# flydog-sdr/FlyDog_SDR_GPS

Measured on AMD Instinct MI355X. Metric: IQ Msamples/s ingested (waterfall + GPS acq); value = GPS acq, BASELINE configs[1], higher is better.
Workload: dtype f32

## Files before the change

### flydog_sdr_gps_amd/_lib.py

```python
import ctypes as C
import os

import numpy as np

_HERE = os.path.dirname(os.path.abspath(__file__))
_LIB = None

ABI_VERSION = 4


class KiwiGpuError(RuntimeError):
    def __init__(self, status, where, text):
        super().__init__("%s failed: %s (status %d)" % (where, text, status))
        self.status = status


def library_path():
    return os.environ.get("KIWIGPU_LIBRARY") or os.path.join(_HERE, "libkiwigpu.so")


class AcqResultC(C.Structure):
    _fields_ = [("snr", C.c_float), ("dop", C.c_int32), ("idx", C.c_int32), ("valid", C.c_int32)]


# ... 253 lines not shown
    "kg_rxbank_set_wf": (_i, [_vp, _i, C.c_uint64, _i, _i]),
    "kg_rxbank_set_wf_pkt": (_i, [_vp, _i, C.c_uint32, C.c_uint32, _i]),
    "kg_rxbank_set_unpack": (_i, [_vp, C.c_float, C.c_float, C.c_float, _i]),
    "kg_rxbank_step": (_i, [_vp, _vp, _vp, _vp]),
    "kg_rxbank_adc_done": (_i, [_vp, _vp, _i]),
    "kg_snd_iq_payload_dev": (_i, [_vp, _vp, _i, _vp, _sz, _i, _i, _vp, _sz]),
    "kg_rxbank_set_little_endian": (_i, [_vp, _i, _i]),
    "kg_post_get_mode": (_i, [_vp, _i]),
    "kg_math_dev": (_i, [_vp, _i, C.c_float, _vp, C.c_uint32, C.c_size_t, _vp]),
    "kg_math_atan2f_dev": (_i, [_vp, _vp, _vp, C.c_size_t, _vp]),
    "kg_rxbank_poll": (_i, [_vp]),
    "kg_rxbank_ready": (_i, [_vp]),
    "kg_rxbank_join": (_i, [_vp, _i]),
    "kg_rxbank_leave": (_i, [_vp, _i]),
    "kg_rxbank_is_active": (_i, [_vp, _i]),
    "kg_rxbank_audio_map": (_i, [_vp, _vp, _vp, _vp, _vp]),
    "kg_fir_process_each_dev": (_i, [_vp, _vp, _i, _vp, _sz, _vp, _vp, _sz, _vp]),
    "kg_rxbank_sync": (_i, [_vp]),
    "kg_rxbank_frame_map": (_i, [_vp, _vp, _vp, _vp]),
    "kg_rxbank_buffers": (_i, [_vp, _vp]),
    "kg_rxbank_host_profile": (_i, [_vp, C.c_char_p, _sz]),
    "kg_acq_debug_fft_stamps": (_i, [_vp, _i, _vp, _i]),
    "kg_acq_debug_corr_stamps": (_i, [_vp, _i, _vp, _i, _vp, _i]),
}


def _share_hip_runtime_with_torch():
    import sys
    if "torch" in sys.modules or os.environ.get("KIWIGPU_NO_TORCH_PRELOAD") == "1":
        return
    import importlib.util
    if importlib.util.find_spec("torch") is not None:
        try:
            import torch
        except Exception as e:
            import warnings
            warnings.warn("kiwigpu: torch is installed but failed to import (%s: %s); libkiwigpu.so will use "
                          "the system HIP runtime" % (type(e).__name__, e))


def load_library():
    global _LIB
    if _LIB is not None:
        return _LIB
    path = library_path()
    if not os.path.exists(path):
# ... 138 lines not shown
```

### flydog_sdr_gps_amd/acq.py

```python
import ctypes as C
from collections import namedtuple

import numpy as np

from . import sats as _sats
from . import prn as _prn
from ._lib import Context, cell_dtype, check, ptr, result_dtype

NSAMPLES = 65536
FFT_LEN = 16384
DECIM = 4
BIN_SIZE = 249.755859375
NSAMPLES_10MS = 163680
FFT_LEN_10MS = 65536
BIN_SIZE_10MS = 4.092e6 / 65536
DOP_LO, DOP_HI = -20, 20
MIN_SIG = 16

AcqResult = namedtuple("AcqResult", "sat snr lo_shift ca_shift valid")


class Searcher:

    def __init__(self, ctx=None, max_sats=_sats.MAX_SATS, dop_lo=DOP_LO, dop_hi=DOP_HI,
# ... 119 lines not shown
        self._last = (int(nblocks), sats.size)

    def fetch(self, want_cells=True):
        nb, ns = self._last
        res = np.zeros((nb, ns), result_dtype)
        cells = np.zeros((nb, ns, self.ndop), cell_dtype) if want_cells else None
        check(self.lib.kg_acq_fetch(self.h, ptr(res), ptr(cells)), "kg_acq_fetch")
        return res, cells

    def correlate_many(self, sats, nblocks=1, want_cells=True, first_block=0):
        self.correlate_async(sats, nblocks, first_block)
        return self.fetch(want_cells)

    def correlate(self, sat, block_data=None):
        if block_data is not None:
            self.set_data_fft(block_data, 0)
        res, _ = self.correlate_many([sat], 1, want_cells=False)
        r = res[0, 0]
        return float(r["snr"]), int(r["dop"]), int(r["idx"]), int(r["valid"])

    def results_dev(self):
        return self.lib.kg_acq_results_dev(self.h)

    def search(self, sats, packed=None, iq16=None, lo_shift=0, ca_shift=0):
        if packed is not None:
            self.sample(packed)
        elif iq16 is not None:
            self.sample_iq16(iq16)
        res, _ = self.correlate_many(list(sats), 1, want_cells=False)
        out = []
        for sat, r in zip(sats, res[0]):
            if r["valid"]:
                lo_shift, ca_shift = int(r["dop"]), int(r["idx"]) * DECIM
            out.append(AcqResult(int(sat), float(r["snr"]), lo_shift, ca_shift, int(r["valid"])))
        return out
```

### flydog_sdr_gps_amd/csrc/kg_acq.hip

```cpp
#include "kg_common.h"
#include "kg_fft.h"
#include "kg_acq_tables.h"

#include <math.h>
#include <stdlib.h>
#include <vector>

#define SUB      4096
#define NTAPS    31
#define DECIM    4


enum { SRC_BITS = 0, SRC_IQ16 = 1, SRC_CHIPS = 2 };

__constant__ float c_hb_even[16] = {
    -0.010233f,  0.010668f, -0.016324f,  0.024377f, -0.036482f,  0.056990f, -0.101993f,
     0.316926f,  0.316926f, -0.101993f,  0.056990f, -0.036482f,  0.024377f, -0.016324f,
     0.010668f, -0.010233f,
};
#define HB_CENTRE 0.500009f

KG_DEV float bipolar(int bit) { return bit ? -1.0f : 1.0f; }

template <int SRC>
KG_DEV cf acq_source(const void *__restrict__ src, int i, int nvalid, int nchips, int boc)
// ... 149 lines not shown
    }
}

struct acq_red { float p; int i; float s; int pad; };

#define ACQ_CLAIM_STRIDE 32
#define ACQ_LDS_BYTES (2 * SUB * sizeof(float2) + 16)

struct __attribute__((aligned(16))) acq_part { float p; int i; float s; int pad; };

struct acq_pair_desc {
    int data_off;
    int code_off;
    int limit;
    int out;
};

struct acq_cell_desc { int data_off, code_off, dop, limit, out; };

struct acq_walk {
    int npairs;
    int ndop, dop_lo;
};

template <int P, bool STAMPS = false>
__global__ __launch_bounds__(256, 2) void acq_correlate_kernel(
    const float2 *__restrict__ data,
    const float2 *__restrict__ code,
    const float2 *__restrict__ tab4096, const float2 *__restrict__ tabN,
    const float2 *__restrict__ comb,
    const acq_pair_desc *__restrict__ pairs,
    int *__restrict__ claim,
    acq_walk walk,
    int halo,
    acq_part *__restrict__ parts,
    unsigned long long *__restrict__ stamps = nullptr)
{
    static_assert(P == 4 || P == 16, "N = 16384 or 65536");
    constexpr int LOGP = P == 4 ? 2 : 4;
    extern __shared__ __attribute__((aligned(16))) float2 smem[];
    float2 *tileA = smem, *tileB = smem + SUB;
    typedef __attribute__((address_space(3))) volatile int acq_lds_int;
    acq_lds_int *claim_slot = (acq_lds_int *) (smem + 2 * SUB);
    const int t = threadIdx.x;
    unsigned long long *st = (STAMPS && t == 0 && blockIdx.x == 8) ? stamps : nullptr;
    if (STAMPS && st) { st[0] = __builtin_amdgcn_s_memtime(); st[1] = __builtin_amdgcn_s_memrealtime(); }
    unsigned long long *wgt = (STAMPS && t == 0) ? stamps + 512 + 4 * blockIdx.x : nullptr;
    int wg_cells = 0;
    if (STAMPS && wgt) {
        wgt[0] = __builtin_amdgcn_s_memrealtime();
        wgt[2] = (unsigned long long) __builtin_amdgcn_s_getreg((20 << 0) | (0 << 6) | (31 << 11));
    }

    kg_tw4096 tw;
    kg_tw4096_load(tw, tab4096, t);
    cf V[4];
#pragma unroll
    for (int dd = 0; dd < 4; dd++) V[dd] = kg_ld(&tabN[t + 1024 * dd]);

    const int xcd = blockIdx.x & 7, slot = blockIdx.x >> 3, nslots = gridDim.x >> 3;
    const int gpairs = (walk.npairs - xcd + 7) >> 3;
    const bool spread = walk.npairs < 8;
    const int ndop = walk.ndop, ncell = spread ? (walk.npairs * ndop - xcd + 7) >> 3 : gpairs * ndop;

    typedef unsigned u4 __attribute__((ext_vector_type(4)));
    const int rowb_c = 2 * (256 + 2 * halo) * (int) sizeof(float2);
    const int plane_c = 8 * 2 * (256 + 2 * halo);
    cf d[16], c[16];
    struct acq_rsrc { __amdgpu_buffer_rsrc_t drs, crs; int dvo, cvo; };
    auto fetch_prepare = [&](int data_off, int code_off, int dop, int k2) {
        const int s = k2 - dop;
        const int q0 = s >> LOGP;
        acq_rsrc r;
        r.drs = __builtin_amdgcn_make_buffer_rsrc(
            (void *) (data + data_off + k2 * SUB), 0, SUB * (int) sizeof(float2), 0x00020000);
        r.crs = __builtin_amdgcn_make_buffer_rsrc(
            (void *) (code + code_off + (s & (P - 1)) * plane_c), 0, plane_c * (int) sizeof(float2), 0x00020000);
        r.dvo = t * 16; r.cvo = (t + q0 + halo) * 16;
        return r;
    };
    auto fetch_row = [&](const acq_rsrc &r, int i) {
        const u4 dv = __builtin_amdgcn_raw_buffer_load_b128(r.drs, r.dvo, i * 4096, 0);
        const u4 cv = __builtin_amdgcn_raw_buffer_load_b128(r.crs, r.cvo, i * rowb_c, 0);
        d[2 * i] = cf{__uint_as_float(dv[0]), __uint_as_float(dv[1])};
// ... 1 lines not shown
        c[2 * i] = cf{__uint_as_float(cv[0]), __uint_as_float(cv[1])};
        c[2 * i + 1] = cf{__uint_as_float(cv[2]), __uint_as_float(cv[3])};
    };
    auto fetch_drow = [&](const acq_rsrc &r, int i) {
        int so;
        asm volatile("s_mov_b32 %0, %1" : "=s"(so) : "i"(i * 4096));
        const u4 dv = __builtin_amdgcn_raw_buffer_load_b128(r.drs, r.dvo, so, 0);
        d[2 * i] = cf{__uint_as_float(dv[0]), __uint_as_float(dv[1])};
        d[2 * i + 1] = cf{__uint_as_float(dv[2]), __uint_as_float(dv[3])};
    };
    auto fetch_crow = [&](const acq_rsrc &r, int i) {
        const u4 cv = __builtin_amdgcn_raw_buffer_load_b128(r.crs, r.cvo, i * rowb_c, 0);
        c[2 * i] = cf{__uint_as_float(cv[0]), __uint_as_float(cv[1])};
        c[2 * i + 1] = cf{__uint_as_float(cv[2]), __uint_as_float(cv[3])};
    };
    auto fetch = [&](int data_off, int code_off, int dop, int k2) {
        const acq_rsrc r = fetch_prepare(data_off, code_off, dop, k2);
#pragma unroll
        for (int i = 0; i < 8; i++) fetch_row(r, i);
    };
    auto describe = [&](int idx) {
        const int cell = spread ? (idx << 3) + xcd : idx;
        const int pg = cell / ndop, di = cell - pg * ndop;
        const acq_pair_desc pd = pairs[spread ? pg : (pg << 3) + xcd];
        return acq_cell_desc{pd.data_off, pd.code_off, walk.dop_lo + di, pd.limit, pd.out + di};
    };

    int cur_idx = slot, nxt_idx = slot + nslots;
    if (cur_idx >= ncell) return;
    acq_cell_desc cur = describe(cur_idx);
    fetch(cur.data_off, cur.code_off, cur.dop, P - 1);

    if (t == 0) claim_slot[1] = slot + 2 * nslots;
    int par = 0;

    int st_item = 0;
    for (;;) {
        const bool more = nxt_idx < ncell;
        const acq_cell_desc nxt = describe(more ? nxt_idx : cur_idx);
        int claimed = 0;
        if (t == 0) claimed = __hip_atomic_fetch_add(&claim[xcd * ACQ_CLAIM_STRIDE], 1, __ATOMIC_RELAXED, __HIP_MEMORY_SCOPE_AGENT);
        cf acc[16];
        cf yprev[16];
        auto accumulate = [&](cf (&yv)[16], bool first, bool mid = false) {
            if (first) {
#pragma unroll
                for (int m = 0; m < 16; m++) acc[m] = yv[m];
// ... 120 lines not shown
                    bp = take ? pw : bp; br = take ? m : br;
                    sum += pw;
                } else {
                    const bool in = t + 256 * m < limit, take = in & (pw > bp);
                    bp = take ? pw : bp; br = take ? m : br;
                    sum += in ? pw : 0.f;
                }
            }
            bi = t + 256 * br;
        }
        {
            float wmax = bp, wsum = sum;
            kg_wave_max_sum(wmax, wsum);
            const int wn = kg_wave_min(bp == wmax ? bi : 0x7fffffff);
            if ((t & 63) == 0) parts[4 * cur.out + (t >> 6)] = acq_part{wmax, wn, wsum, 0};
        }
        if (t == 0) claim_slot[par] = 3 * nslots + claimed;
        const int nn_idx = __builtin_amdgcn_readfirstlane(claim_slot[par ^ 1]);
        par ^= 1;
        if (STAMPS) wg_cells++;
        if (!more) break;
        cur = nxt; cur_idx = nxt_idx; nxt_idx = nn_idx;
    }
    if (STAMPS && st) { st[2] = __builtin_amdgcn_s_memtime(); st[3] = __builtin_amdgcn_s_memrealtime(); }
    if (STAMPS && wgt) { wgt[1] = __builtin_amdgcn_s_memrealtime(); wgt[3] = (unsigned long long) wg_cells; }
}

#define ACQ8_LDS_BYTES (3 * SUB * sizeof(float2) + 8 * sizeof(acq_red) + 16 + 16 * 8 * sizeof(float2) + 3 * 512 * 4)


template <int P, bool STAMPS = false>
__global__ __launch_bounds__(512, 1) void acq_correlate8_kernel(
    const float2 *__restrict__ data, const float2 *__restrict__ code,
    const float2 *__restrict__ tab4096, const float2 *__restrict__ tabN,
    const float2 *__restrict__ comb8,
    const float2 *__restrict__ quart,
    const acq_pair_desc *__restrict__ pairs, int *__restrict__ claim, acq_walk walk, int halo,
    kg_acq_cell *__restrict__ cells, unsigned long long *__restrict__ stamps = nullptr)
{
    static_assert(P == 4 || P == 16, "N = 16384 or 65536");
    constexpr int LOGP = P == 4 ? 2 : 4;
    extern __shared__ __attribute__((aligned(16))) float2 smem[];
    float2 *tile0 = smem, *tile1 = smem + SUB, *tile2 = smem + 2 * SUB;
    acq_red *red = (acq_red *) (smem + 3 * SUB);
    volatile int *red_claim = (volatile int *) (red + 8);
    float2 *cst = (float2 *) ((char *) (red + 8) + 16);
// ... 274 lines not shown
        int bi = i + 512 * (int) __builtin_ctz(rowmask | 0x80000000u);
        KG_STAMP(STAMPS, stc, 1);
        xch_p[i] = bp; xch_i[i] = bi; xch_s[i] = sum;
        KG_STAMP(STAMPS, stc, 2);
        if (i == 448) *red_claim = 2 * nslots + claimed;
        __syncthreads();
        KG_STAMP(STAMPS, stc, 3);
        const int nn_idx = __builtin_amdgcn_readfirstlane(*red_claim);
        prev_out = cur.out; prev_limit = limit;
        if (!more) {
            reduce_pairs();
            __syncthreads();
            merge_store(prev_out, prev_limit);
        }
        KG_STAMP(STAMPS, stc, 4);
        if (!more) break;
        cur = nxt; cur_idx = nxt_idx; nxt_idx = nn_idx;
    }
}

__global__ __launch_bounds__(64) void acq_select_kernel(kg_acq_cell *__restrict__ cells, const acq_part *__restrict__ parts,
                                                       const acq_pair_desc *__restrict__ pairs, int np1,
                                                       int npairs, int dop_lo, int ndop,
                                                       kg_acq_result *__restrict__ out, int *__restrict__ claim)
{
    const int q = blockIdx.x, lane = threadIdx.x;
    if (q == 0 && lane < 16) claim[lane * ACQ_CLAIM_STRIDE] = 0;
    if (q >= npairs) return;
    const acq_pair_desc pd = pairs[q];
    const int p = pd.out / ndop;
    float bs = 0.f;
    int bd = 0x7fffffff, bidx = 0;
    for (int di = lane; di < ndop; di += 64) {
        kg_acq_cell c;
        if (q < np1) {
            const acq_part *w = parts + 4 * ((size_t) pd.out + di);
            acq_part a = w[0], b = w[2];
            const acq_part a1 = w[1], b1 = w[3];
            auto merge = [](acq_part &x, const acq_part &o) {
                const bool take = (o.p > x.p) | ((o.p == x.p) & (o.i < x.i));
                x.p = take ? o.p : x.p; x.i = take ? o.i : x.i;
                x.s += o.s;
            };
            merge(a, a1); merge(b, b1); merge(a, b);
            const float ave = a.s / (float) pd.limit;
            c.snr = a.p / ave;
            c.max_pwr = a.p; c.tot_pwr = a.s; c.idx = a.i;
            cells[(size_t) pd.out + di] = c;
        } else {
            c = cells[(size_t) pd.out + di];
// ... 40 lines not shown
    kg_dbuf<float2> d_fsub;
    kg_dbuf<float2> d_fsub_code;
    kg_dbuf<uint8_t> d_in;
    kg_hbuf<uint8_t> h_pin[4];
    hipEvent_t ev_pin[4];
    int pin_next;
    kg_hbuf<uint8_t> h_batch; size_t batch_cap; hipEvent_t ev_batch;
    hipStream_t cstream; hipEvent_t ev_in_free; bool in_free_set;
    kg_dbuf<uint8_t> d_chips;
    kg_dbuf<kg_acq_cell> d_cells;
    kg_dbuf<acq_part> d_parts;
    kg_dbuf<kg_acq_result> d_results;
    kg_dbuf<int> d_claim;
    std::vector<int> limits, code_set;
    std::vector<int> last_sats;
    const acq_pair_desc *d_pairs1, *d_pairs4;
    unsigned long pairs_seq;
    int last_first, last_nblocks, last_nsats, np1, np4, table_nblocks;
    hipStream_t fstream;
    bool own_fstream;
    std::vector<hipEvent_t> ev_ready, ev_done;
    std::vector<int> ready_of, done_of;
    int grid1;
};

static inline __host__ __device__ size_t plane_pos(int k1, int halo_col, int H, int layout)
{
    if (layout == 0) {
        const int t = k1 & 255, j = k1 >> 8, row = 2 * (256 + 2 * H);
        return (size_t) (j >> 1) * row + 2 * (t + halo_col + H) + (j & 1);
    }
    const int t = k1 & 511, j = k1 >> 9, row = 2 * (512 + 2 * H);
    return (size_t) (j >> 1) * row + 2 * (t + halo_col + H) + (j & 1);
}
static inline size_t spec_len(int P, int H) { return (size_t) P * 8 * 2 * (256 + 2 * H); }
static inline __host__ __device__ size_t plane_len(int H, int layout) { return layout == 0 ? (size_t) 8 * 2 * (256 + 2 * H) : (size_t) 4 * 2 * (512 + 2 * H); }

__global__ void acq_code_overrun_kernel(float2 *__restrict__ dst, int layout_dst, const float2 *__restrict__ src, int layout_src, int P, int H)
{
    const int t = blockIdx.x * blockDim.x + threadIdx.x;
    if (t >= P * H) return;
    const int k2 = t % P, k1 = t / P;
    const float2 v = src ? src[(size_t) k2 * plane_len(H, layout_src) + plane_pos(k1, 0, H, layout_src)] : make_float2(0.f, 0.f);
    const int T = layout_dst == 0 ? 256 : 512, J = SUB / T;
    dst[(size_t) k2 * plane_len(H, layout_dst) + plane_pos(k1 + T * (J - 1), T, H, layout_dst)] = v;
}

// ... 91 lines not shown
        KG_TRY(a->d_comb8.alloc(comb8.size(), "kg_acq_create: combine constants"));
        KG_HIP(hipMemcpy(a->d_comb8, comb8.data(), sizeof(float2) * comb8.size(), hipMemcpyHostToDevice));
    }
    KG_TRY(a->d_code.alloc(a->code_len * max_sats, "kg_acq_create: code spectra"));
    KG_TRY(a->d_data.alloc((size_t) N * max_blocks, "kg_acq_create: data spectra"));
    KG_TRY(a->d_td.alloc((size_t) N * max_blocks, "kg_acq_create: decimated samples"));
    KG_TRY(a->d_td_code.alloc(N, "kg_acq_create: decimated samples"));
    KG_TRY(a->d_fsub.alloc((size_t) N * max_blocks, "kg_acq_create: sub-transforms"));
    KG_TRY(a->d_fsub_code.alloc(N, "kg_acq_create: sub-transforms"));
    KG_TRY(a->d_in.alloc(a->in_stride * max_blocks, "kg_acq_create: input staging"));
    for (int k = 0; k < 4; k++) {
        KG_TRY(a->h_pin[k].alloc(a->in_stride, "kg_acq_create: pinned input slots"));
        KG_HIP(hipEventCreateWithFlags(&a->ev_pin[k], hipEventDisableTiming));
    }
    KG_HIP(hipEventCreateWithFlags(&a->ev_batch, hipEventDisableTiming));
    KG_HIP(hipEventCreateWithFlags(&a->ev_in_free, hipEventDisableTiming));
    KG_TRY(kg_stream_get(ctx->device, &a->cstream));
    KG_TRY(a->d_chips.alloc(8192, "kg_acq_create: chips"));
    KG_TRY(a->d_cells.alloc((size_t) max_blocks * max_sats * a->ndop, "kg_acq_create: cells"));
    KG_TRY(a->d_parts.alloc(4 * (size_t) max_blocks * max_sats * a->ndop, "kg_acq_create: wave records"));
    KG_TRY(a->d_results.alloc((size_t) max_blocks * max_sats, "kg_acq_create: results"));
    KG_TRY(a->d_claim.alloc(16 * ACQ_CLAIM_STRIDE, "kg_acq_create: claim counters"));
    KG_HIP(hipMemset(a->d_claim, 0, sizeof(int) * 16 * ACQ_CLAIM_STRIDE));
    {
        const char *e = kg_tuning_env("KIWIGPU_ACQ_FRONT_STREAM");
        if (e && e[0] == '1') {
            KG_TRY(kg_stream_get(ctx->device, &a->fstream));
            a->own_fstream = true;
        }
    }
    a->ready_of.assign(max_blocks, -1); a->done_of.assign(max_blocks, -1);
    a->ev_ready.reserve(max_blocks); a->ev_done.reserve(max_blocks);
    for (int b = 0; b < max_blocks; b++) {
        hipEvent_t e1, e2;
        KG_HIP(hipEventCreateWithFlags(&e1, hipEventDisableTiming));
        a->ev_ready.push_back(e1);
        KG_HIP(hipEventCreateWithFlags(&e2, hipEventDisableTiming));
        a->ev_done.push_back(e2);
    }
    KG_HIP(hipMemset(a->d_data, 0, spec * max_blocks));
    KG_HIP(hipFuncSetAttribute((const void *) acq_fft_sub_kernel<false>,
                               hipFuncAttributeMaxDynamicSharedMemorySize, 2 * SUB * sizeof(float2)));
    KG_HIP(hipFuncSetAttribute((const void *) acq_fft_sub_kernel<true>,
                               hipFuncAttributeMaxDynamicSharedMemorySize, 2 * SUB * sizeof(float2)));
    int occ1 = 0;
#define ACQ_SETUP(PP)                                                                                          \
// ... 369 lines not shown
int kg_acq_get_data_td(kg_acq *a, int block, float *td)
{
    int rc = check_block(a, block, td, "kg_acq_get_data_td");
    if (rc) return rc;
    KG_HIP(hipStreamSynchronize(a->fstream));
    KG_HIP(hipMemcpyAsync(td, a->d_td + (size_t) block * a->fft_len, sizeof(float2) * a->fft_len,
                          hipMemcpyDeviceToHost, a->ctx->stream));
    KG_HIP(hipStreamSynchronize(a->ctx->stream));
    return KG_OK;
}

}

template <int P, bool STAMPS>
static void launch_correlate(kg_acq *a, hipStream_t st, int first, const acq_pair_desc *d_pairs, int npairs,
                             unsigned long long *d_stamps)
{
    const int grid = a->grid1;
    const acq_walk w = {npairs, a->ndop, a->dop_lo};
    hipLaunchKernelGGL((acq_correlate_kernel<P, STAMPS>), dim3(grid), dim3(256), ACQ_LDS_BYTES, st,
                       (const float2 *) (a->d_data + (size_t) first * a->fft_len), (const float2 *) a->d_code,
                       (const float2 *) a->ctx->d_tab4096, (const float2 *) a->d_tabN,
                       (const float2 *) a->d_comb, d_pairs,
                       a->d_claim, w, a->halo, a->d_parts, d_stamps);
}

extern "C" {

int kg_acq_correlate_blocks_async(kg_acq *a, int first, int nblocks, const int *sats, int nsats)
{
    KG_REQUIRE(a && sats, KG_ERR_INVALID, "kg_acq_correlate_async: null argument");
    int rc = kg_ctx_use(a->ctx);
    if (rc) return rc;
    KG_REQUIRE(nblocks >= 1 && first >= 0 && first + nblocks <= a->max_blocks, KG_ERR_INVALID,
               "kg_acq_correlate_async: blocks %d..%d (max %d)", first, first + nblocks - 1,
               a->max_blocks);
    KG_REQUIRE(nsats >= 1 && nsats <= a->max_sats, KG_ERR_INVALID,
               "kg_acq_correlate_async: nsats %d (max %d)", nsats, a->max_sats);
    hipStream_t st = a->ctx->stream;
    bool same = (int) a->last_sats.size() == nsats && a->table_nblocks == nblocks &&
                a->ctx->ring_next - a->pairs_seq < KG_RING_SLOTS / 2;
    for (int i = 0; same && i < nsats; i++) same = a->last_sats[i] == sats[i];
    if (!same) {
        for (int i = 0; i < nsats; i++) {
            KG_REQUIRE(sats[i] >= 0 && sats[i] < a->max_sats, KG_ERR_INVALID,
                       "kg_acq_correlate_async: sats[%d] = %d out of range", i, sats[i]);
            KG_REQUIRE(a->code_set[sats[i]], KG_ERR_STATE,
                       "kg_acq_correlate_async: no code set for sat %d", sats[i]);
        }
        std::vector<acq_pair_desc> tab[2];
        for (int blk = 0; blk < nblocks; blk++)
            for (int i = 0; i < nsats; i++) {
                const int sat = sats[i];
                acq_pair_desc pd;
                pd.data_off = blk * a->fft_len;
                pd.code_off = (int) (sat * a->code_len);
                pd.limit = a->limits[sat];
                pd.out = (blk * nsats + i) * a->ndop;
                tab[a->limits[sat] <= SUB ? 0 : 1].push_back(pd);
            }
        a->np1 = (int) tab[0].size(); a->np4 = (int) tab[1].size();
        tab[0].insert(tab[0].end(), tab[1].begin(), tab[1].end());
        void *d = nullptr;
        KG_TRY(kg_ctx_stage(a->ctx, tab[0].data(), sizeof(acq_pair_desc) * tab[0].size(), &d));
        a->d_pairs1 = (const acq_pair_desc *) d;
        a->d_pairs4 = a->d_pairs1 + a->np1;
        a->pairs_seq = a->ctx->ring_next;
        a->last_sats.assign(sats, sats + nsats);
        a->table_nblocks = nblocks;
        if (sizeof(acq_pair_desc) * tab[0].size() > KG_RING_SLOT_BYTES) a->last_sats.clear();
    }
    if (a->own_fstream && (rc = wait_once(st, a->ev_ready, a->ready_of, first, nblocks)) != KG_OK) return rc;
    if (a->np1 > 0) {
        if (a->P == 4) launch_correlate<4, false>(a, st, first, a->d_pairs1, a->np1, nullptr);
        else launch_correlate<16, false>(a, st, first, a->d_pairs1, a->np1, nullptr);
        KG_HIP(hipGetLastError());
    }
    if (a->np4 > 0) {
        KG_REQUIRE(a->d_data_b != nullptr, KG_ERR_STATE, "kg_acq_correlate_async: a long-window code without its layout of the data spectra");
        const acq_walk w = {a->np4, a->ndop, a->dop_lo};
        if (a->P == 4)
            hipLaunchKernelGGL(acq_correlate8_kernel<4>, dim3(a->grid8), dim3(512), ACQ8_LDS_BYTES, st,
                               (const float2 *) (a->d_data_b + (size_t) first * a->fft_len), (const float2 *) a->d_code,
                               (const float2 *) a->ctx->d_tab4096, (const float2 *) a->d_tabN, (const float2 *) a->d_comb8,
                               (const float2 *) a->d_quart, a->d_pairs4, a->d_claim + 8 * ACQ_CLAIM_STRIDE, w, a->halo, a->d_cells);
        else
            hipLaunchKernelGGL(acq_correlate8_kernel<16>, dim3(a->grid8), dim3(512), ACQ8_LDS_BYTES, st,
                               (const float2 *) (a->d_data_b + (size_t) first * a->fft_len), (const float2 *) a->d_code,
                               (const float2 *) a->ctx->d_tab4096, (const float2 *) a->d_tabN, (const float2 *) a->d_comb8,
                               (const float2 *) a->d_quart, a->d_pairs4, a->d_claim + 8 * ACQ_CLAIM_STRIDE, w, a->halo, a->d_cells);
        KG_HIP(hipGetLastError());
    }
    const int npairs = nblocks * nsats;
    hipLaunchKernelGGL(acq_select_kernel, dim3(npairs), dim3(64), 0, st,
                       a->d_cells, (const acq_part *) a->d_parts, a->d_pairs1, a->np1, npairs, a->dop_lo, a->ndop,
                       a->d_results, a->d_claim);
    KG_HIP(hipGetLastError());
    if (a->own_fstream) {
        KG_HIP(hipEventRecord(a->ev_done[first], st));
        for (int b = first; b < first + nblocks; b++) a->done_of[b] = first;
    }
    a->last_first = first; a->last_nblocks = nblocks; a->last_nsats = nsats;
    return KG_OK;
}

int kg_acq_correlate_async(kg_acq *a, int nblocks, const int *sats, int nsats)
{
    return kg_acq_correlate_blocks_async(a, 0, nblocks, sats, nsats);
}

int kg_acq_fetch(kg_acq *a, kg_acq_result *results, kg_acq_cell *cells)
{
    KG_REQUIRE(a && results, KG_ERR_INVALID, "kg_acq_fetch: null argument");
    int rc = kg_ctx_use(a->ctx);
    if (rc) return rc;
    KG_REQUIRE(a->last_nsats > 0, KG_ERR_STATE, "kg_acq_fetch: nothing was launched");
    const size_t np = (size_t) a->last_nblocks * a->last_nsats;
    hipStream_t st = a->ctx->stream;
    KG_HIP(hipMemcpyAsync(results, a->d_results, sizeof(kg_acq_result) * np, hipMemcpyDeviceToHost, st));
    if (cells)
        KG_HIP(hipMemcpyAsync(cells, a->d_cells, sizeof(kg_acq_cell) * np * a->ndop, hipMemcpyDeviceToHost, st));
    KG_HIP(hipStreamSynchronize(st));
    return KG_OK;
}

int kg_acq_correlate(kg_acq *a, int nblocks, const int *sats, int nsats, kg_acq_result *results,
                     kg_acq_cell *cells)
{
    int rc = kg_acq_correlate_async(a, nblocks, sats, nsats);
    if (rc) return rc;
    return kg_acq_fetch(a, results, cells);
}

void *kg_acq_results_dev(kg_acq *a) { return a ? (void *) a->d_results : nullptr; }

int kg_acq_debug_corr_stamps(kg_acq *a, int nblocks, const int *sats, int nsats,
                             unsigned long long *stamps, int n)
{
    KG_REQUIRE(a && stamps && n >= 512 + 4 * 1024, KG_ERR_INVALID, "kg_acq_debug_corr_stamps: need 4608 slots");
    int rc = kg_acq_correlate_async(a, nblocks, sats, nsats);
    if (rc) return rc;
    hipStream_t st = a->ctx->stream;
    if (a->np1 == 0 && a->np4 > 0) {
        unsigned long long *d = nullptr;
        const size_t bytes = sizeof(unsigned long long) * (512 + 4 * 1024);
        kg_scope tmp(a->ctx);
        KG_TRY(tmp.alloc(&d, 512 + 4 * 1024, "kg_acq_debug_corr_stamps"));
        KG_HIP(hipMemset(d, 0, bytes));
        KG_HIP(hipMemsetAsync(a->d_claim, 0, sizeof(int) * 16 * ACQ_CLAIM_STRIDE, st));
        const acq_walk w = {a->np4, a->ndop, a->dop_lo};
        if (a->P == 4) {
            KG_HIP(hipFuncSetAttribute((const void *) acq_correlate8_kernel<4, true>,
                                       hipFuncAttributeMaxDynamicSharedMemorySize, ACQ8_LDS_BYTES));
            hipLaunchKernelGGL((acq_correlate8_kernel<4, true>), dim3(a->grid8), dim3(512), ACQ8_LDS_BYTES, st,
                               (const float2 *) a->d_data_b, (const float2 *) a->d_code, (const float2 *) a->ctx->d_tab4096,
                               (const float2 *) a->d_tabN, (const float2 *) a->d_comb8, (const float2 *) a->d_quart,
                               a->d_pairs4, a->d_claim + 8 * ACQ_CLAIM_STRIDE, w, a->halo, a->d_cells, d);
// ... 61 lines not shown
```

### include/kiwigpu.h

```cpp
#ifndef KIWIGPU_H
#define KIWIGPU_H

#include <stddef.h>
#include <stdint.h>

#ifdef __cplusplus
extern "C" {
#endif

#define KG_ABI_VERSION 4

typedef enum {
    KG_OK = 0,
    KG_ERR_NO_DEVICE = -1,
    KG_ERR_INVALID = -2,
    KG_ERR_HIP = -3,
    KG_ERR_NOMEM = -4,
    KG_ERR_STATE = -5
} kg_status;

const char *kg_strerror(int status);
const char *kg_last_error(void);
int kg_abi_version(void);

// ... 471 lines not shown
    uint32_t last_ms;
    int32_t reserved;
    double fi, fft_sec, time;
} kg_fftext_info;
int kg_fftext_create(kg_ctx *ctx, int nchan, kg_fftext **out);
void kg_fftext_destroy(kg_fftext *fx);
int kg_fftext_set_rate(kg_fftext *fx, double sample_rate);
int kg_fftext_set_run(kg_fftext *fx, int ch, int run, int is_sam, int is_qam);
int kg_fftext_set_itime(kg_fftext *fx, int ch, double itime);
int kg_fftext_clear(kg_fftext *fx, int ch);
int kg_fftext_restart(kg_fftext *fx, int ch);
int kg_fftext_process_dev(kg_fftext *fx, const int32_t *chans, int nch, const int32_t *nblk, const int32_t *inst, const float *d_spec,
                          size_t spec_stride, uint8_t *d_rows, size_t row_stride, int max_rows, int32_t *rx_of_row, int32_t *ent_of_row,
                          int32_t *blk_of_row, int32_t *bin_of_row);
int kg_fftext_process(kg_fftext *fx, const int32_t *chans, int nch, const int32_t *nblk, const int32_t *inst, const float *spec,
                      size_t spec_stride, uint8_t *rows, size_t row_stride, int max_rows, int32_t *rx_of_row, int32_t *ent_of_row,
                      int32_t *blk_of_row, int32_t *bin_of_row);
int kg_fftext_due(kg_fftext *fx, int ch, uint32_t now_ms);
int kg_fftext_state(kg_fftext *fx, int ch, kg_fftext_info *info, float *pwr, int32_t *ncma);

int kg_acq_debug_fft_stamps(kg_acq *acq, int block, unsigned long long *stamps, int n);
int kg_acq_debug_corr_stamps(kg_acq *acq, int nblocks, const int *sats, int nsats,
                             unsigned long long *stamps, int n);

typedef struct kg_rxbank kg_rxbank;

int kg_rxbank_create(int device, int nrx, size_t adc_samples_per_step, int rx_mode, kg_rxbank **out);
void kg_rxbank_destroy(kg_rxbank *bank);
kg_ctx *kg_rxbank_ctx(kg_rxbank *bank);
kg_ddc *kg_rxbank_ddc(kg_rxbank *bank);
kg_wf *kg_rxbank_wf(kg_rxbank *bank);
kg_rxddc *kg_rxbank_rxddc(kg_rxbank *bank);
kg_fir *kg_rxbank_fir(kg_rxbank *bank);
kg_post *kg_rxbank_post(kg_rxbank *bank);
kg_adpcm *kg_rxbank_adpcm(kg_rxbank *bank);
kg_nb *kg_rxbank_nb(kg_rxbank *bank);
int kg_rxbank_set_nb_algo(kg_rxbank *bank, int rx, int algo);
int kg_rxbank_nbw_select(kg_rxbank *bank, int rx);
int kg_rxbank_set_nb_enable(kg_rxbank *bank, int rx, int type, int en);
int kg_rxbank_set_nb_param(kg_rxbank *bank, int rx, int type, int param, float pval, float frate);
int kg_rxbank_set_nb_gate(kg_rxbank *bank, int rx, int nb, int th, float frate);
int kg_rxbank_nb_cmd_state(kg_rxbank *bank, int rx, int32_t *ints, float *flts);
int kg_rxbank_set_spec(kg_rxbank *bank, int rx, int n);
kg_fir *kg_rxbank_null_fir(kg_rxbank *bank);
int kg_rxbank_spec_max(kg_rxbank *bank);
int kg_rxbank_spec_map(kg_rxbank *bank, int32_t *rx_of_row, int32_t *inst_of_row, int32_t *blk_of_row);
// ... 56 lines not shown
```

Measured before the change: 2719.

## Deal C/A acquisition pairs to XCD groups by measured per-group speed

Result: no change. 2728, median of 6 (+0.3%).

```diff
diff --git a/flydog_sdr_gps_amd/_lib.py b/flydog_sdr_gps_amd/_lib.py
--- a/flydog_sdr_gps_amd/_lib.py
+++ b/flydog_sdr_gps_amd/_lib.py
@@ -299,6 +299,8 @@
     "kg_rxbank_host_profile": (_i, [_vp, C.c_char_p, _sz]),
     "kg_acq_debug_fft_stamps": (_i, [_vp, _i, _vp, _i]),
     "kg_acq_debug_corr_stamps": (_i, [_vp, _i, _vp, _i, _vp, _i]),
+    "kg_acq_debug_deal": (_i, [_vp, _vp]),
+    "kg_acq_debug_deal_record": (_i, [_vp, _vp, _i]),
 }
 
 
diff --git a/flydog_sdr_gps_amd/acq.py b/flydog_sdr_gps_amd/acq.py
--- a/flydog_sdr_gps_amd/acq.py
+++ b/flydog_sdr_gps_amd/acq.py
@@ -165,6 +165,18 @@
     def results_dev(self):
         return self.lib.kg_acq_results_dev(self.h)
 
+    def debug_deal(self, weights=None):
+        w = None if weights is None else np.ascontiguousarray(weights, np.float64)
+        if w is not None and w.size != 8:
+            raise ValueError("need 8 weights")
+        check(self.lib.kg_acq_debug_deal(self.h, ptr(w)), "kg_acq_debug_deal")
+
+    def debug_deal_record(self):
+        r = np.zeros(20, np.uint64)
+        check(self.lib.kg_acq_debug_deal_record(self.h, ptr(r), r.size), "kg_acq_debug_deal_record")
+        return {"gen": int(r[0]), "start": int(r[1]), "end": r[2:10].astype(np.int64), "cells": r[10:18].astype(np.int64),
+                "npairs": int(r[18])}
+
     def search(self, sats, packed=None, iq16=None, lo_shift=0, ca_shift=0):
         if packed is not None:
             self.sample(packed)
diff --git a/flydog_sdr_gps_amd/csrc/kg_acq.hip b/flydog_sdr_gps_amd/csrc/kg_acq.hip
--- a/flydog_sdr_gps_amd/csrc/kg_acq.hip
+++ b/flydog_sdr_gps_amd/csrc/kg_acq.hip
@@ -1,6 +1,7 @@
 #include "kg_common.h"
 #include "kg_fft.h"
 #include "kg_acq_tables.h"
+#include "kg_acq_deal.h"
 
 #include <math.h>
 #include <stdlib.h>
@@ -196,6 +197,15 @@
     int npairs;
     int ndop, dop_lo;
 };
+struct acq_deal { int base[KG_ACQ_GROUPS], count[KG_ACQ_GROUPS]; };
+#define ACQ_STAMP_START 1
+#define ACQ_STAMP_END 2
+struct acq_feedback { unsigned long long *rec; unsigned long long gen; int cells[KG_ACQ_GROUPS]; int npairs; };
+#define ACQ_FB_LIFE 0
+#define ACQ_FB_CELLS 8
+#define ACQ_FB_START 16
+#define ACQ_FB_NPAIRS 17
+#define ACQ_FB_WORDS 18
 
 template <int P, bool STAMPS = false>
 __global__ __launch_bounds__(256, 2) void acq_correlate_kernel(
@@ -205,7 +215,7 @@
     const float2 *__restrict__ comb,
     const acq_pair_desc *__restrict__ pairs,
     int *__restrict__ claim,
-    acq_walk walk,
+    acq_walk walk, acq_deal deal,
     int halo,
     acq_part *__restrict__ parts,
     unsigned long long *__restrict__ stamps = nullptr)
@@ -233,7 +243,9 @@
     for (int dd = 0; dd < 4; dd++) V[dd] = kg_ld(&tabN[t + 1024 * dd]);
 
     const int xcd = blockIdx.x & 7, slot = blockIdx.x >> 3, nslots = gridDim.x >> 3;
-    const int gpairs = (walk.npairs - xcd + 7) >> 3;
+    const int gbase = deal.base[xcd], gpairs = deal.count[xcd];
+    unsigned long long *const gstamp = (unsigned long long *) (claim + xcd * ACQ_CLAIM_STRIDE);
+    if (t == 0) __hip_atomic_fetch_min(gstamp + ACQ_STAMP_START, (unsigned long long) __builtin_amdgcn_s_memrealtime(), __ATOMIC_RELAXED, __HIP_MEMORY_SCOPE_AGENT);
     const bool spread = walk.npairs < 8;
     const int ndop = walk.ndop, ncell = spread ? (walk.npairs * ndop - xcd + 7) >> 3 : gpairs * ndop;
 
@@ -281,7 +293,7 @@
     auto describe = [&](int idx) {
         const int cell = spread ? (idx << 3) + xcd : idx;
         const int pg = cell / ndop, di = cell - pg * ndop;
-        const acq_pair_desc pd = pairs[spread ? pg : (pg << 3) + xcd];
+        const acq_pair_desc pd = pairs[spread ? pg : gbase + pg];
         return acq_cell_desc{pd.data_off, pd.code_off, walk.dop_lo + di, pd.limit, pd.out + di};
     };
 
@@ -448,6 +460,7 @@
         if (!more) break;
         cur = nxt; cur_idx = nxt_idx; nxt_idx = nn_idx;
     }
+    if (t == 0) __hip_atomic_fetch_max(gstamp + ACQ_STAMP_END, (unsigned long long) __builtin_amdgcn_s_memrealtime(), __ATOMIC_RELAXED, __HIP_MEMORY_SCOPE_AGENT);
     if (STAMPS && st) { st[2] = __builtin_amdgcn_s_memtime(); st[3] = __builtin_amdgcn_s_memrealtime(); }
     if (STAMPS && wgt) { wgt[1] = __builtin_amdgcn_s_memrealtime(); wgt[3] = (unsigned long long) wg_cells; }
 }
@@ -768,10 +781,30 @@
 __global__ __launch_bounds__(64) void acq_select_kernel(kg_acq_cell *__restrict__ cells, const acq_part *__restrict__ parts,
                                                        const acq_pair_desc *__restrict__ pairs, int np1,
                                                        int npairs, int dop_lo, int ndop,
-                                                       kg_acq_result *__restrict__ out, int *__restrict__ claim)
+                                                       kg_acq_result *__restrict__ out, int *__restrict__ claim, acq_feedback fb)
 {
     const int q = blockIdx.x, lane = threadIdx.x;
     if (q == 0 && lane < 16) claim[lane * ACQ_CLAIM_STRIDE] = 0;
+    if (q == 0 && fb.rec) {
+        unsigned long long *stamp = (unsigned long long *) (claim + (lane & 7) * ACQ_CLAIM_STRIDE);
+        const unsigned long long s = stamp[ACQ_STAMP_START], e = stamp[ACQ_STAMP_END];
+        unsigned long long first = s;
+#pragma unroll
+        for (int off = 4; off >= 1; off >>= 1) {
+            const unsigned long long o = __shfl_xor(first, off);
+            first = o < first ? o : first;
+        }
+        const unsigned long long life = (first != ~0ull && e > first) ? (e - first < 0xffffffffull ? e - first : 0xffffffffull) : 0;
+        const unsigned long long tag = fb.gen << 32;
+        volatile unsigned long long *rec = fb.rec;
+        if (lane < 8) {
+            rec[ACQ_FB_LIFE + lane] = tag | life;
+            rec[ACQ_FB_CELLS + lane] = tag | (unsigned) fb.cells[lane];
+            stamp[ACQ_STAMP_START] = ~0ull; stamp[ACQ_STAMP_END] = 0;
+        }
+        if (lane == 8) rec[ACQ_FB_START] = tag | (first & 0xffffffffull);
+        if (lane == 9) rec[ACQ_FB_NPAIRS] = tag | (unsigned) fb.npairs;
+    }
     if (q >= npairs) return;
     const acq_pair_desc pd = pairs[q];
     const int p = pd.out / ndop;
@@ -858,7 +891,24 @@
     std::vector<hipEvent_t> ev_ready, ev_done;
     std::vector<int> ready_of, done_of;
     int grid1;
+    kg_hbuf<unsigned long long> h_rec;
+    unsigned long long launch_gen;
+    kg_acq_dealer dealer;
+    int deal_mode;
+    double forced_w[KG_ACQ_GROUPS];
+    int deal_count[KG_ACQ_GROUPS], deal_npairs;
+    acq_deal deal;
 };
+enum { ACQ_DEAL_EVEN = 0, ACQ_DEAL_SPEED = 1, ACQ_DEAL_FORCED = 2 };
+#define ACQ_DEAL_DEFAULT ACQ_DEAL_SPEED
+static int acq_own_deal_mode()
+{
+    if (const char *e = kg_tuning_env("KIWIGPU_ACQ_DEAL")) {
+        if (!strcmp(e, "even")) return ACQ_DEAL_EVEN;
+        if (!strcmp(e, "speed")) return ACQ_DEAL_SPEED;
+    }
+    return ACQ_DEAL_DEFAULT;
+}
 
 static inline __host__ __device__ size_t plane_pos(int k1, int halo_col, int H, int layout)
 {
@@ -996,6 +1046,15 @@
     KG_TRY(a->d_results.alloc((size_t) max_blocks * max_sats, "kg_acq_create: results"));
     KG_TRY(a->d_claim.alloc(16 * ACQ_CLAIM_STRIDE, "kg_acq_create: claim counters"));
     KG_HIP(hipMemset(a->d_claim, 0, sizeof(int) * 16 * ACQ_CLAIM_STRIDE));
+    for (int x = 0; x < KG_ACQ_GROUPS; x++) {
+        const unsigned long long none = ~0ull;
+        KG_HIP(hipMemcpy((unsigned long long *) (a->d_claim + x * ACQ_CLAIM_STRIDE) + ACQ_STAMP_START, &none, sizeof none, hipMemcpyHostToDevice));
+    }
+    KG_TRY(a->h_rec.alloc(KG_ACQ_REC_WORDS, "kg_acq_create: dealer record"));
+    memset(a->h_rec, 0, sizeof(unsigned long long) * KG_ACQ_REC_WORDS);
+    a->launch_gen = 0; a->deal_npairs = -1;
+    kg_acq_dealer_init(&a->dealer);
+    a->deal_mode = acq_own_deal_mode();
     {
         const char *e = kg_tuning_env("KIWIGPU_ACQ_FRONT_STREAM");
         if (e && e[0] == '1') {
@@ -1411,7 +1470,43 @@
                        (const float2 *) (a->d_data + (size_t) first * a->fft_len), (const float2 *) a->d_code,
                        (const float2 *) a->ctx->d_tab4096, (const float2 *) a->d_tabN,
                        (const float2 *) a->d_comb, d_pairs,
-                       a->d_claim, w, a->halo, a->d_parts, d_stamps);
+                       a->d_claim, w, a->deal, a->halo, a->d_parts, d_stamps);
+}
+
+static bool acq_read_record(const kg_acq *a, unsigned long long *r)
+{
+    const volatile unsigned long long *h = a->h_rec;
+    unsigned long long w[ACQ_FB_WORDS];
+    for (int i = 0; i < ACQ_FB_WORDS; i++) w[i] = h[i];
+    const unsigned long long g32 = w[0] >> 32;
+    for (int i = 1; i < ACQ_FB_WORDS; i++)
+        if (w[i] >> 32 != g32) return false;
+    if (g32 == 0) return false;
+    unsigned long long gen = (a->launch_gen & ~0xffffffffull) | g32;
+    if (gen > a->launch_gen) gen = gen >= (1ull << 32) ? gen - (1ull << 32) : 0;
+    const unsigned long long start = (1ull << 32) | (w[ACQ_FB_START] & 0xffffffffull);
+    r[KG_ACQ_REC_GEN0] = r[KG_ACQ_REC_GEN1] = gen;
+    r[KG_ACQ_REC_START] = start;
+    for (int x = 0; x < KG_ACQ_GROUPS; x++) {
+        r[KG_ACQ_REC_END + x] = start + (w[ACQ_FB_LIFE + x] & 0xffffffffull);
+        r[KG_ACQ_REC_CELLS + x] = w[ACQ_FB_CELLS + x] & 0xffffffffull;
+    }
+    r[KG_ACQ_REC_NPAIRS] = w[ACQ_FB_NPAIRS] & 0xffffffffull;
+    return gen != 0;
+}
+
+static void acq_choose_deal(kg_acq *a, int n1, int *count)
+{
+    if (a->deal_mode == ACQ_DEAL_SPEED) {
+        unsigned long long r[KG_ACQ_REC_WORDS];
+        if (acq_read_record(a, r)) kg_acq_deal_observe(&a->dealer, r);
+    }
+    if (n1 < KG_ACQ_GROUPS || a->deal_mode == ACQ_DEAL_EVEN) kg_acq_deal_even(n1, count);
+    else if (a->deal_mode == ACQ_DEAL_FORCED) kg_acq_deal_quantise(n1, a->forced_w, count);
+    else kg_acq_deal_decide(&a->dealer, n1, a->deal_count, a->deal_npairs == n1, count);
+    int sum = 0;
+    for (int x = 0; x < KG_ACQ_GROUPS; x++) sum += count[x] < 0 ? n1 + 1 : count[x];
+    if (sum != n1) kg_acq_deal_even(n1, count);
 }
 
 extern "C" {
@@ -1430,13 +1525,21 @@
     bool same = (int) a->last_sats.size() == nsats && a->table_nblocks == nblocks &&
                 a->ctx->ring_next - a->pairs_seq < KG_RING_SLOTS / 2;
     for (int i = 0; same && i < nsats; i++) same = a->last_sats[i] == sats[i];
+    int n1 = a->np1;
     if (!same) {
+        n1 = 0;
         for (int i = 0; i < nsats; i++) {
             KG_REQUIRE(sats[i] >= 0 && sats[i] < a->max_sats, KG_ERR_INVALID,
                        "kg_acq_correlate_async: sats[%d] = %d out of range", i, sats[i]);
             KG_REQUIRE(a->code_set[sats[i]], KG_ERR_STATE,
                        "kg_acq_correlate_async: no code set for sat %d", sats[i]);
-        }
+            if (a->limits[sats[i]] <= SUB) n1 += nblocks;
+        }
+    }
+    int count[KG_ACQ_GROUPS];
+    acq_choose_deal(a, n1, count);
+    if (a->deal_npairs != n1 || memcmp(count, a->deal_count, sizeof count)) same = false;
+    if (!same) {
         std::vector<acq_pair_desc> tab[2];
         for (int blk = 0; blk < nblocks; blk++)
             for (int i = 0; i < nsats; i++) {
@@ -1449,12 +1552,24 @@
                 tab[a->limits[sat] <= SUB ? 0 : 1].push_back(pd);
             }
         a->np1 = (int) tab[0].size(); a->np4 = (int) tab[1].size();
+        KG_REQUIRE(a->np1 == n1, KG_ERR_STATE, "kg_acq_correlate_async: %d C/A pairs counted, %d listed", n1, a->np1);
+        kg_acq_deal_even(n1, a->deal.count);
+        for (int x = 0, b = 0; x < KG_ACQ_GROUPS; b += a->deal.count[x++]) a->deal.base[x] = b;
+        if (n1 >= KG_ACQ_GROUPS) {
+            std::vector<int> order(n1);
+            std::vector<acq_pair_desc> own(tab[0]);
+            memcpy(a->deal.count, count, sizeof count);
+            kg_acq_deal_layout(n1, count, a->deal.base, order.data());
+            for (int i = 0; i < n1; i++) tab[0][i] = own[order[i]];
+        }
+        a->deal_npairs = -1;
         tab[0].insert(tab[0].end(), tab[1].begin(), tab[1].end());
         void *d = nullptr;
         KG_TRY(kg_ctx_stage(a->ctx, tab[0].data(), sizeof(acq_pair_desc) * tab[0].size(), &d));
         a->d_pairs1 = (const acq_pair_desc *) d;
         a->d_pairs4 = a->d_pairs1 + a->np1;
         a->pairs_seq = a->ctx->ring_next;
+        memcpy(a->deal_count, count, sizeof count); a->deal_npairs = n1;
         a->last_sats.assign(sats, sats + nsats);
         a->table_nblocks = nblocks;
         if (sizeof(acq_pair_desc) * tab[0].size() > KG_RING_SLOT_BYTES) a->last_sats.clear();
@@ -1481,9 +1596,16 @@
         KG_HIP(hipGetLastError());
     }
     const int npairs = nblocks * nsats;
+    acq_feedback fb = {nullptr, 0, {0, 0, 0, 0, 0, 0, 0, 0}, 0};
+    if (a->np1 > 0) {
+        const bool spread = a->np1 < KG_ACQ_GROUPS;
+        fb.rec = a->h_rec; fb.gen = ++a->launch_gen & 0xffffffffull; fb.npairs = spread ? 0 : a->np1;
+        for (int x = 0; x < KG_ACQ_GROUPS; x++)
+            fb.cells[x] = spread ? (a->np1 * a->ndop - x + 7) >> 3 : a->deal.count[x] * a->ndop;
+    }
     hipLaunchKernelGGL(acq_select_kernel, dim3(npairs), dim3(64), 0, st,
                        a->d_cells, (const acq_part *) a->d_parts, a->d_pairs1, a->np1, npairs, a->dop_lo, a->ndop,
-                       a->d_results, a->d_claim);
+                       a->d_results, a->d_claim, fb);
     KG_HIP(hipGetLastError());
     if (a->own_fstream) {
         KG_HIP(hipEventRecord(a->ev_done[first], st));
@@ -1522,6 +1644,30 @@
 }
 
 void *kg_acq_results_dev(kg_acq *a) { return a ? (void *) a->d_results : nullptr; }
+
+int kg_acq_debug_deal(kg_acq *a, const double *weights)
+{
+    KG_REQUIRE(a, KG_ERR_INVALID, "kg_acq_debug_deal: null argument");
+    if (!weights) {
+        a->deal_mode = acq_own_deal_mode();
+        return KG_OK;
+    }
+    double ideal[KG_ACQ_GROUPS];
+    KG_REQUIRE(kg_acq_deal_ideal(1, weights, ideal), KG_ERR_INVALID, "kg_acq_debug_deal: weights must be finite, >= 0 and not all zero");
+    memcpy(a->forced_w, weights, sizeof a->forced_w);
+    a->deal_mode = ACQ_DEAL_FORCED;
+    return KG_OK;
+}
+
+int kg_acq_debug_deal_record(kg_acq *a, unsigned long long *rec, int n)
+{
+    KG_REQUIRE(a && rec && n >= KG_ACQ_REC_WORDS, KG_ERR_INVALID, "kg_acq_debug_deal_record: need %d slots", KG_ACQ_REC_WORDS);
+    int rc = kg_ctx_use(a->ctx);
+    if (rc) return rc;
+    KG_HIP(hipStreamSynchronize(a->ctx->stream));
+    if (!acq_read_record(a, rec)) memset(rec, 0, sizeof(unsigned long long) * KG_ACQ_REC_WORDS);
+    return KG_OK;
+}
 
 int kg_acq_debug_corr_stamps(kg_acq *a, int nblocks, const int *sats, int nsats,
                              unsigned long long *stamps, int n)
diff --git a/flydog_sdr_gps_amd/csrc/kg_acq_deal.h b/flydog_sdr_gps_amd/csrc/kg_acq_deal.h
--- /dev/null
+++ b/flydog_sdr_gps_amd/csrc/kg_acq_deal.h
@@ -0,0 +1,126 @@
+#pragma once
+
+#include <math.h>
+#include <string.h>
+
+#define KG_ACQ_GROUPS 8
+
+#define KG_ACQ_DEAL_MIN_PER_GROUP 25
+#define KG_ACQ_DEAL_MAX_RATIO 1.25
+#define KG_ACQ_DEAL_ALPHA 0.25
+#define KG_ACQ_DEAL_KEEP 0.75
+
+#define KG_ACQ_REC_GEN0 0
+#define KG_ACQ_REC_START 1
+#define KG_ACQ_REC_END 2
+#define KG_ACQ_REC_CELLS 10
+#define KG_ACQ_REC_NPAIRS 18
+#define KG_ACQ_REC_GEN1 19
+#define KG_ACQ_REC_WORDS 20
+
+struct kg_acq_dealer {
+    double speed[KG_ACQ_GROUPS];
+    unsigned long long last_gen;
+    int nobs;
+};
+
+static inline void kg_acq_dealer_init(kg_acq_dealer *d) { memset(d, 0, sizeof *d); }
+
+static inline void kg_acq_deal_even(int npairs, int *count)
+{
+    for (int x = 0; x < KG_ACQ_GROUPS; x++) count[x] = (npairs - x + 7) >> 3;
+}
+
+static inline int kg_acq_deal_ideal(int npairs, const double *w, double *ideal)
+{
+    double sum = 0.0;
+    for (int x = 0; x < KG_ACQ_GROUPS; x++) {
+        if (!(w[x] >= 0.0) || !isfinite(w[x])) return 0;
+        sum += w[x];
+    }
+    if (!(sum > 0.0) || !isfinite(sum)) return 0;
+    for (int x = 0; x < KG_ACQ_GROUPS; x++) ideal[x] = (double) npairs * (w[x] / sum);
+    return 1;
+}
+
+static inline void kg_acq_deal_quantise(int npairs, const double *w, int *count)
+{
+    double ideal[KG_ACQ_GROUPS], frac[KG_ACQ_GROUPS];
+    if (npairs < 0 || !kg_acq_deal_ideal(npairs, w, ideal)) { kg_acq_deal_even(npairs < 0 ? 0 : npairs, count); return; }
+    int given = 0;
+    for (int x = 0; x < KG_ACQ_GROUPS; x++) {
+        count[x] = (int) floor(ideal[x]);
+        if (count[x] > npairs) count[x] = npairs;
+        frac[x] = ideal[x] - count[x];
+        given += count[x];
+    }
+    for (; given < npairs; given++) {
+        int best = 0;
+        for (int x = 1; x < KG_ACQ_GROUPS; x++)
+            if (frac[x] > frac[best]) best = x;
+        count[best]++; frac[best] -= 1.0;
+    }
+    for (int x = KG_ACQ_GROUPS - 1; given > npairs && x >= 0; x--)
+        while (given > npairs && count[x] > 0) { count[x]--; given--; }
+}
+
+static inline int kg_acq_deal_observe(kg_acq_dealer *d, const unsigned long long *rec)
+{
+    const unsigned long long gen = rec[KG_ACQ_REC_GEN1];
+    if (gen == 0 || gen != rec[KG_ACQ_REC_GEN0] || gen <= d->last_gen) return 0;
+    d->last_gen = gen;
+    const unsigned long long start = rec[KG_ACQ_REC_START], np = rec[KG_ACQ_REC_NPAIRS];
+    if (start == 0 || start == ~0ull || np < (unsigned long long) KG_ACQ_GROUPS * KG_ACQ_DEAL_MIN_PER_GROUP || np > (1ull << 30)) return 0;
+    double rate[KG_ACQ_GROUPS], lo = 0.0, hi = 0.0, mean = 0.0;
+    for (int x = 0; x < KG_ACQ_GROUPS; x++) {
+        const unsigned long long end = rec[KG_ACQ_REC_END + x], cells = rec[KG_ACQ_REC_CELLS + x];
+        if (end <= start || end - start > 1000000000ull || cells == 0 || cells > (1ull << 40)) return 0;
+        rate[x] = (double) cells / (double) (end - start);
+        lo = x == 0 || rate[x] < lo ? rate[x] : lo;
+        hi = x == 0 || rate[x] > hi ? rate[x] : hi;
+        mean += rate[x] / KG_ACQ_GROUPS;
+    }
+    if (!(lo > 0.0) || hi > KG_ACQ_DEAL_MAX_RATIO * lo) return 0;
+    const double a = d->nobs == 0 ? 1.0 : KG_ACQ_DEAL_ALPHA;
+    for (int x = 0; x < KG_ACQ_GROUPS; x++) d->speed[x] += a * (rate[x] / mean - d->speed[x]);
+    d->nobs++;
+    return 1;
+}
+
+static inline int kg_acq_deal_decide(const kg_acq_dealer *d, int npairs, const int *cur, int cur_valid, int *count)
+{
+    double ideal[KG_ACQ_GROUPS];
+    int cur_sum = 0;
+    for (int x = 0; cur_valid && x < KG_ACQ_GROUPS; x++) cur_sum += cur[x];
+    if (cur_valid && cur_sum != npairs) cur_valid = 0;
+    if (npairs < KG_ACQ_GROUPS * KG_ACQ_DEAL_MIN_PER_GROUP || d->nobs == 0 || !kg_acq_deal_ideal(npairs, d->speed, ideal))
+        kg_acq_deal_even(npairs, count);
+    else {
+        bool keep = cur_valid != 0;
+        for (int x = 0; keep && x < KG_ACQ_GROUPS; x++) keep = fabs((double) cur[x] - ideal[x]) <= KG_ACQ_DEAL_KEEP;
+        if (keep) memcpy(count, cur, sizeof(int) * KG_ACQ_GROUPS);
+        else kg_acq_deal_quantise(npairs, d->speed, count);
+    }
+    if (!cur_valid) return 1;
+    return memcmp(count, cur, sizeof(int) * KG_ACQ_GROUPS) != 0;
+}
+
+static inline void kg_acq_deal_layout(int npairs, const int *count, int *base, int *order)
+{
+    int own[KG_ACQ_GROUPS], give_from[KG_ACQ_GROUPS], b = 0;
+    kg_acq_deal_even(npairs, own);
+    for (int x = 0; x < KG_ACQ_GROUPS; x++) {
+        base[x] = b; b += count[x];
+        give_from[x] = count[x] < own[x] ? count[x] : own[x];
+    }
+    int gx = 0, gi = give_from[0];
+    for (int x = 0; x < KG_ACQ_GROUPS; x++) {
+        int *o = order + base[x];
+        const int keep = count[x] < own[x] ? count[x] : own[x];
+        for (int i = 0; i < keep; i++) o[i] = x + KG_ACQ_GROUPS * i;
+        for (int i = keep; i < count[x]; i++) {
+            while (gx < KG_ACQ_GROUPS && gi >= own[gx]) { gx++; gi = gx < KG_ACQ_GROUPS ? give_from[gx] : 0; }
+            o[i] = gx + KG_ACQ_GROUPS * gi++;
+        }
+    }
+}
diff --git a/include/kiwigpu.h b/include/kiwigpu.h
--- a/include/kiwigpu.h
+++ b/include/kiwigpu.h
@@ -517,6 +517,8 @@
 int kg_acq_debug_fft_stamps(kg_acq *acq, int block, unsigned long long *stamps, int n);
 int kg_acq_debug_corr_stamps(kg_acq *acq, int nblocks, const int *sats, int nsats,
                              unsigned long long *stamps, int n);
+int kg_acq_debug_deal(kg_acq *acq, const double *weights);
+int kg_acq_debug_deal_record(kg_acq *acq, unsigned long long *rec, int n);
 
 typedef struct kg_rxbank kg_rxbank;
 
```
